# AnnSeidel/genometools

Measured on AMD Instinct MI355X. Metric: Gbp/s ESA build (suf+lcp+bwt), 3 Gbp DNA, 1/2/4/8 MI355X; bit-exact vs CPU, higher is better.
Workload: dtype u64; 1 GPU; human-like DNA (2% N, 24 seqs, repeats) n=3000000000 seed=43 -suf -lcp -bwt (BASELINE.json configs[2]); parallelism=1 device, pair_suffixes=341032298, tied_suffixes=390540711, refine_rounds=9, maxbranchdepth=8256

## Files before the change

genometools_amd/csrc/esa_engine.hip:

```cpp
#include <stdarg.h>
#include <stdlib.h>
#include <chrono>
#include <functional>
#include <type_traits>
#include <vector>
#include "../../include/gtamd_esa.h"
#include "esa_prims.h"
#include "esa_devutil.h"

static thread_local char g_err[1024] = "";
void gtamd_set_error(const char *fmt, ...) {
  va_list ap;
  va_start(ap, fmt);
  vsnprintf(g_err, sizeof g_err, fmt, ap);
  va_end(ap);
}
extern "C" const char *gtamd_esa_last_error(void) { return g_err; }

extern "C" int gtamd_device_count(void) {
  GTAMD_ABI_BEGIN
  int n = 0;
  if (hipGetDeviceCount(&n) != hipSuccess) return 0;
  return n;
  GTAMD_ABI_END(0)
// ... 570 lines not shown
                              u32 numparts, u64 nblocks, u32 *__restrict__ counts) {
  const u32 r = threadIdx.x;
  if (r >= numparts) return;
  const u64 first = (u64) r * nblocks, last = first + nblocks - 1;
  counts[r] = boff[last] + bcount[last] - boff[first];
}

struct Tiles {
  u64 T;
  u32 self;
  __device__ __forceinline__ u32 owner(u64 q, u64 *off) const {
    const u64 d = q / T;
    *off = q - d * T;
    return (u32) d;
  }
};

struct OwnerOfKey {
  const u64 *keys;
  const u32 *vals;
  const u8 *owner;
  u64 *keys_out;
  u32 *vals_out;
  __device__ __forceinline__ u32 dest(u64 j) const {
    return owner[keys[j] >> (64 - PART_BITS)];
  }
  __device__ __forceinline__ void local(u64) const {}
  __device__ __forceinline__ void emit(u64 j, u32 at) const {
    keys_out[at] = keys[j];
    vals_out[at] = vals[j];
  }
};

template <typename P> struct InitialRanks {
  const P *sa;
  const u64 *tiebits;
  const u32 *carry;
  u64 c0, index_offset;
  Tiles tl;
  P *isa;
  u32 *srec;
  const u32 *sel;
  int wb;
  __device__ __forceinline__ u32 dest(u64 j) const {
    u64 off;
    const u64 p = (u64) sa[c0 + j];
    if (sel != nullptr) {
      const u64 w = p >> wb;
      if (!((sel[w >> 5] >> (w & 31)) & 1u)) return DEST_NONE;
    }
    const u32 d = tl.owner(p, &off);
    return d == tl.self ? DEST_LOCAL : d;
  }
  __device__ __forceinline__ P rank_of(u64 i) const {
    const u64 w = i >> 6;
    const int b = (int) (i & 63);
    const u64 below = b == 63 ? ~0ull : ((2ull << b) - 1ull);
    const u64 z = ~tiebits[w] & below;
    const u64 head = z ? w * 64 + (u64) (63 - __clzll((long long) z)) : (u64) carry[w];
    return (P) (index_offset + head);
  }
  __device__ __forceinline__ void local(u64 j) const {
    u64 off;
    (void) tl.owner((u64) sa[c0 + j], &off);
    isa[off] = rank_of(c0 + j);
  }
  __device__ __forceinline__ void emit(u64 j, u32 at) const {
    u64 off;
    (void) tl.owner((u64) sa[c0 + j], &off);
    const u64 r = (u64) rank_of(c0 + j);
    u32 *rec = srec + (u64) at * (1 + sizeof(P) / 4);
    rec[0] = (u32) off;
    rec[1] = (u32) r;
    if (sizeof(P) == 8) rec[2] = (u32) (r >> 32);
  }
};

template <typename P> struct FilteredRanks {
  const P *fpos;
  const u32 *fhead;
  u64 index_offset;
  Tiles tl;
  P *isa;
  u32 *srec;
  static constexpr int RANKREC = 1 + (int) (sizeof(P) / 4);
  __device__ __forceinline__ u32 dest(u64 j) const {
    u64 off;
    const u32 d = tl.owner((u64) fpos[j], &off);
    return d == tl.self ? DEST_LOCAL : d;
  }
  __device__ __forceinline__ void local(u64 j) const {
    u64 off;
    (void) tl.owner((u64) fpos[j], &off);
// ... 427 lines not shown
__global__ __launch_bounds__(256) void k_unres_emit(
    const u64 *__restrict__ tiebits, u64 nwords, const u32 *__restrict__ blkoff,
    const u32 *__restrict__ carry, const P *__restrict__ sa,
    u32 *__restrict__ uidx0, u32 *__restrict__ uidx, P *__restrict__ upos,
    u32 *__restrict__ ugrp) {
  __shared__ u32 s_scan[4];
  const u64 w = (u64) blockIdx.x * 256 + threadIdx.x;
  u64 t = 0, u = 0;
  if (w < nwords) {
    t = tiebits[w];
    const u64 nx = w + 1 < nwords ? tiebits[w + 1] : 0ull;
    u = t | (t >> 1) | (nx << 63);
  }
  u32 tot;
  u32 j = blkoff[blockIdx.x] + block_scan_excl_sum((u32) __popcll(u), &tot, s_scan);
  if (u == 0) return;
  const u32 carryw = carry[w];
  while (u) {
    const int b = __ffsll((unsigned long long) u) - 1;
    u &= u - 1;
    const u64 i = w * 64 + b;
    const u64 below = b == 63 ? ~0ull : ((2ull << b) - 1ull);
    const u64 z = ~t & below;
    uidx0[j] = (u32) i;
    uidx[j] = (u32) i;
    upos[j] = sa[i];
    ugrp[j] = z ? (u32) (w * 64 + (63 - __clzll((long long) z))) : carryw;
    j++;
  }
}

__global__ __launch_bounds__(256) void k_heads(
    const u64 *__restrict__ tiebits, const u32 *__restrict__ carry, u64 N,
    u32 rank_offset, u32 *__restrict__ heads) {
  const u64 i0 = ((u64) blockIdx.x * 256 + threadIdx.x) * 4;
  if (i0 >= N) return;
  const u64 t = tiebits[i0 >> 6];
  u32 h[4];
  h[0] = group_head(tiebits, carry, i0);
#pragma unroll
  for (int g = 1; g < 4; g++)
    h[g] = ((t >> ((i0 + g) & 63)) & 1ull) ? h[g - 1] : (u32) (i0 + g);
  if (i0 + 4 <= N) {
    *reinterpret_cast<uint4 *>(heads + i0) =
        make_uint4(rank_offset + h[0], rank_offset + h[1], rank_offset + h[2],
                   rank_offset + h[3]);
  } else {
    for (int g = 0; g < 4 && i0 + g < N; g++) heads[i0 + g] = rank_offset + h[g];
  }
}

constexpr int RW_BITS = 15;
constexpr int RW_THREADS = 1024;

__global__ __launch_bounds__(RW_THREADS) void k_rank_window(
    const u32 *__restrict__ pos, const u32 *__restrict__ heads, u64 N, int wb,
    int split, u32 nbuckets, u32 *__restrict__ rank, const u32 *__restrict__ winlist,
    int fb, u32 nfine, u64 M) {
  __shared__ u32 s_win[1 << RW_BITS];
  u32 bucket = blockIdx.x, half = 0;
  if (split == 2) {
    bucket = (blockIdx.x >> 4) * 8u + (blockIdx.x & 7u);
    half = (blockIdx.x >> 3) & 1u;
  }
  if (bucket >= nbuckets) return;
  const int sb = wb - (split == 2 ? 1 : 0);
  const u32 smask = (1u << sb) - 1u;
  const u64 first = (u64) bucket << wb;
  const u64 total = winlist != nullptr ? M : N;
  const u64 end = first + (1ull << wb) < total ? first + (1ull << wb) : total;
  const u64 cnt = end - first;
  const u32 *bp = pos + first, *bh = heads + first;
  const u64 cnt4 = (wb >= 2) ? (cnt & ~3ull) : 0;
  for (u64 i = (u64) threadIdx.x * 4; i < cnt4; i += (u64) RW_THREADS * 4) {
    const uint4 p4 = *reinterpret_cast<const uint4 *>(bp + i);
// ... 97 lines not shown
}

constexpr int WF_THREADS = 1024;
constexpr int WF_Q = 4;
constexpr u64 WF_SPAN = (u64) WF_THREADS * 4 * WF_Q;
constexpr int WF_ITER = 8;
constexpr int WF_QUEUE = 2048;
constexpr u64 WF_LDS_MAX = 60 * 1024;
template <typename P>
__device__ __forceinline__ void wf_load4(const P *__restrict__ sa, u64 i0, u64 NL, P v[4]) {
  if (i0 + 4 <= NL) {
    if (sizeof(P) == 4) {
      const uint4 x = *reinterpret_cast<const uint4 *>(sa + i0);
      v[0] = (P) x.x; v[1] = (P) x.y; v[2] = (P) x.z; v[3] = (P) x.w;
    } else {
      const ulonglong2 v0 = *reinterpret_cast<const ulonglong2 *>(sa + i0);
      const ulonglong2 v1 = *reinterpret_cast<const ulonglong2 *>(sa + i0 + 2);
      v[0] = (P) v0.x; v[1] = (P) v0.y; v[2] = (P) v1.x; v[3] = (P) v1.y;
    }
  } else {
#pragma unroll
    for (int k = 0; k < 4; k++) v[k] = i0 + k < NL ? sa[i0 + k] : (P) 0;
  }
}
template <typename P>
static size_t wf_lds_bytes(u64 nww, bool lsel) {
  const u64 nww4 = (nww + 3) & ~3ull;
  return (size_t) ((lsel ? nww4 * 4 + nww4 : 0) + 16 + WF_QUEUE * (sizeof(P) + 2));
}
template <typename P, bool LSEL>
__global__ __launch_bounds__(WF_THREADS) __attribute__((amdgpu_waves_per_eu(8, 8))) void k_win_filter(
    const P *__restrict__ sa, u64 NL, int wb, const u32 *__restrict__ sel, u32 nww,
    const u32 *__restrict__ pref, const u64 *__restrict__ tiebits, const u32 *__restrict__ carry,
    P *__restrict__ fpos, u32 *__restrict__ fhead, u64 cap, Stats *stats) {
  extern __shared__ __attribute__((aligned(16))) u32 s_dyn[];
  __shared__ u32 s_scan[WF_THREADS / 64];
  __shared__ u32 s_base;
  const u32 nww4 = (nww + 3u) & ~3u;
  u32 *s_sel = s_dyn, *s_pref4 = s_dyn + nww4;
  P *s_qpos = reinterpret_cast<P *>(s_dyn + (LSEL ? nww4 + nww4 / 4 : 0u) + ((LSEL ? nww4 / 4 : 0u) & 1u));
  unsigned short *s_qidx = reinterpret_cast<unsigned short *>(s_qpos + WF_QUEUE);
  if (LSEL) {
    for (u32 i = threadIdx.x; i < nww4; i += WF_THREADS) s_sel[i] = i < nww ? sel[i] : 0u;
    if (pref != nullptr)
      for (u32 i = threadIdx.x; i < nww4 / 4; i += WF_THREADS) s_pref4[i] = pref[4 * i];
    __syncthreads();
  }
  const u32 *selw = LSEL ? s_sel : sel;
  for (int it = 0; it < WF_ITER; it++) {
    const u64 first = ((u64) blockIdx.x * WF_ITER + it) * WF_SPAN;
    if (first >= NL) break;
    P p[WF_Q][4];
#pragma unroll
    for (int q = 0; q < WF_Q; q++)
      wf_load4(sa, first + (u64) q * (WF_THREADS * 4) + (u64) threadIdx.x * 4, NL, p[q]);
    u32 m = 0;
#pragma unroll
    for (int q = 0; q < WF_Q; q++) {
      const u64 i0 = first + (u64) q * (WF_THREADS * 4) + (u64) threadIdx.x * 4;
#pragma unroll
      for (int k = 0; k < 4; k++) {
        const u32 w = (u32) (p[q][k] >> wb);
        if (i0 + k < NL) m |= ((selw[w >> 5] >> (w & 31)) & 1u) << (4 * q + k);
      }
    }
    u32 tot;
    const u32 excl = block_scan_excl<SCAN_SUM, WF_THREADS>((u32) __popc(m), &tot, s_scan);
// ... 8 lines not shown
      for (int q = 0; q < WF_Q; q++) {
#pragma unroll
        for (int k = 0; k < 4; k++)
          if ((m >> (4 * q + k)) & 1u) {
            if (o < (u32) WF_QUEUE) {
              s_qpos[o] = p[q][k];
              s_qidx[o] = (unsigned short) (q * (WF_THREADS * 4) + threadIdx.x * 4 + k);
            }
            o++;
          }
      }
      __syncthreads();
      if (s_base == ~0u) return;
      const u32 nq = tot - r0 < (u32) WF_QUEUE ? tot - r0 : (u32) WF_QUEUE;
      const u64 base = (u64) s_base + r0;
      for (u32 j = threadIdx.x; j < nq; j += WF_THREADS) {
        P v = s_qpos[j];
        if (pref != nullptr) {
          const u32 w = (u32) (v >> wb), x = w >> 5;
          u32 d;
          if (LSEL) {
            const uint4 g = *reinterpret_cast<const uint4 *>(s_sel + (x & ~3u));
            const u32 low = (1u << (w & 31)) - 1u, jj = x & 3u;
            d = s_pref4[x >> 2] + (u32) __popc(g.x & (jj == 0 ? low : ~0u)) +
                (u32) __popc(g.y & (jj == 1 ? low : (jj > 1 ? ~0u : 0u))) +
                (u32) __popc(g.z & (jj == 2 ? low : (jj > 2 ? ~0u : 0u))) +
                (u32) __popc(g.w & (jj == 3 ? low : 0u));
          } else {
            d = pref[x] + (u32) __popc(sel[x] & ((1u << (w & 31)) - 1u));
          }
          v = (P) (((u64) d << wb) | ((u64) v & ((1ull << wb) - 1ull)));
        }
        fpos[base + j] = v;
        fhead[base + j] = group_head(tiebits, carry, first + s_qidx[j]);
      }
      __syncthreads();
    }
  }
}

constexpr int LCP_CHUNK = 32;
constexpr u32 PAIR_SWAP = 1u << 31;

__device__ __forceinline__ u64 pair_heads(u64 t, u64 nx) {
  return ~t & ((t >> 1) | (nx << 63)) & ~((t >> 2) | (nx << 62));
}

__device__ __forceinline__ u64 small_heads(u64 t, u64 nx, int g) {
  u64 m = ~t & ~((t >> g) | (nx << (64 - g)));
  for (int k = 1; k < g; k++) m &= (t >> k) | (nx << (64 - k));
  return m;
}

__global__ __launch_bounds__(256) void k_pair_words(
    const u64 *__restrict__ tiebits, u64 nwords, u32 *__restrict__ cnt,
    u32 *__restrict__ scnt, u32 *__restrict__ rcnt, u64 *__restrict__ tiebits2) {
  __shared__ u32 s4[4];
  const u64 w = (u64) blockIdx.x * 256 + threadIdx.x;
  u32 np = 0, n3 = 0, n4 = 0;
  if (w < nwords) {
    const u64 t = tiebits[w];
    const u64 nx = w + 1 < nwords ? tiebits[w + 1] : 0ull;
    const u64 ph = pair_heads(t, nx);
    u64 prevhead = 0;
    if (w > 0) prevhead = pair_heads(tiebits[w - 1], t) >> 63;
    np = (u32) __popcll(ph);
    n3 = (u32) __popcll(small_heads(t, nx, 3));
// ... 172 lines not shown
  if (w < nwords) {
    const u64 t = tiebits[w];
    const u64 nx = w + 1 < nwords ? tiebits[w + 1] : 0ull;
    ph = pair_heads(t, nx);
  }
  u32 tot;
  u32 local = block_scan_excl_sum((u32) __popcll(ph), &tot, s_scan);
  const u32 base = off[blockIdx.x];
  const bool staged = tot <= (u32) PE_STAGE;
  while (ph) {
    const int b = __ffsll((unsigned long long) ph) - 1;
    ph &= ph - 1;
    const u64 i = w * 64 + b;
    const u64 j = (u64) base + local;
    const P a = sa[i];
    const u64 v = (sizeof(P) == 4 ? (u64) sa[i + 1] : i) | (j << 32);
    if (staged) { s_pk[local] = a; s_pv[local] = v; s_pi[local] = (u32) i; }
    else { pkey[j] = a; pval[j] = v; pidx[j] = (u32) i; }
    local++;
  }
  if (!staged) return;
  __syncthreads();
  for (u32 k = threadIdx.x; k < tot; k += 256) {
    pkey[base + k] = s_pk[k];
    pval[base + k] = s_pv[k];
    pidx[base + k] = s_pi[k];
  }
}

constexpr int PR_LINE = 16;
template <int BITS, typename P>
__global__ __launch_bounds__(256) void k_pair_resolve(
    Text t, const P *__restrict__ pkey, const u64 *__restrict__ pval, u64 nrec, u64 np,
    const u32 *__restrict__ pidx, P *__restrict__ sa, u32 *__restrict__ res, Stats *stats,
    int chunk) {
  __shared__ unsigned long long s_sum[4], s_large[4];
  __shared__ u32 s_max[4];
  const int lane = threadIdx.x & 63, w = threadIdx.x >> 6;
  unsigned long long sum = 0, nlarge = 0;
  u32 mx = 0;
  const u64 nchunks = (nrec + chunk - 1) / chunk;
  for (u64 c = (u64) blockIdx.x * 256 + threadIdx.x; c < nchunks;
       c += (u64) gridDim.x * 256) {
    constexpr int RING = 4;
    u64 ra[RING] = {0, 0, 0, 0}, rb[RING] = {0, 0, 0, 0}, rl[RING] = {0, 0, 0, 0};
    bool rf[RING] = {true, true, true, true};
    int filled = 0;
    for (int e0 = 0; e0 < chunk; e0 += PR_LINE) {
      const u64 s0 = c * chunk + e0;
      if (s0 >= nrec) break;
      P ak[PR_LINE];
      u64 ivk[PR_LINE];
      if (s0 + PR_LINE <= nrec) {
        if (sizeof(P) == 4) {
#pragma unroll
          for (int q = 0; q < PR_LINE / 4; q++) {
            const uint4 v = *reinterpret_cast<const uint4 *>(pkey + s0 + 4 * q);
            ak[4 * q] = (P) v.x; ak[4 * q + 1] = (P) v.y; ak[4 * q + 2] = (P) v.z; ak[4 * q + 3] = (P) v.w;
          }
        } else {
#pragma unroll
          for (int q = 0; q < PR_LINE / 2; q++) {
            const ulonglong2 v = *reinterpret_cast<const ulonglong2 *>(pkey + s0 + 2 * q);
            ak[2 * q] = (P) v.x; ak[2 * q + 1] = (P) v.y;
          }
        }
#pragma unroll
        for (int q = 0; q < PR_LINE / 2; q++) {
// ... 6 lines not shown
          ak[q] = s0 + q < nrec ? pkey[s0 + q] : (P) 0;
          ivk[q] = s0 + q < nrec ? pval[s0 + q] : 0ull;
        }
      }
#pragma unroll
    for (int e = 0; e < PR_LINE; e++) {
      const u64 s = s0 + e;
      if (s >= nrec || e0 + e >= chunk) continue;
      const u64 a = ak[e];
      const u64 iv = ivk[e];
      const u64 j = iv >> 32;
      const u64 b = sizeof(P) == 4 ? (iv & 0xFFFFFFFFull) : (u64) sa[(iv & 0xFFFFFFFFull) + 1];
      u64 l = 0;
      bool a_first = true, known = false;
#pragma unroll
      for (int k = 0; k < RING; k++) {
        if (k < filled && !known) {
          const u64 d = a - ra[k];
          if (b >= rb[k] && b - rb[k] == d && rl[k] >= (u64) Key<BITS>::KNOWN + d) {
            l = rl[k] - d;
            a_first = rf[k];
            known = true;
          }
        }
      }
      if (!known) l = lcp_extend_long<BITS, 4>(t, a, b, (u64) Key<BITS>::KNOWN, &a_first);
#pragma unroll
      for (int k = RING - 1; k > 0; k--) { ra[k] = ra[k - 1]; rb[k] = rb[k - 1]; rl[k] = rl[k - 1]; rf[k] = rf[k - 1]; }
      ra[0] = a; rb[0] = b; rl[0] = l; rf[0] = a_first;
      if (filled < RING) filled++;
      const u32 lv = l < 0x7FFFFFFFull ? (u32) l : 0x7FFFFFFFu;
      res[j] = lv | (a_first ? 0u : PAIR_SWAP);
      if (j < np) {
        if (!a_first) {
          const u64 i = sizeof(P) == 4 ? (u64) pidx[j] : (iv & 0xFFFFFFFFull);
          sa[i] = (P) b;
          sa[i + 1] = (P) a;
        }
        sum += lv;
        nlarge += lv >= GTAMD_LCPOVERFLOW;
        mx = lv > mx ? lv : mx;
      }
    }
    }
  }
#pragma unroll
  for (int d = 32; d >= 1; d >>= 1) {
    sum += __shfl_xor(sum, d, 64);
    nlarge += __shfl_xor(nlarge, d, 64);
    const u32 o = __shfl_xor(mx, d, 64);
    mx = o > mx ? o : mx;
  }
  if (lane == 0) { s_sum[w] = sum; s_large[w] = nlarge; s_max[w] = mx; }
  __syncthreads();
  if (threadIdx.x == 0) {
    unsigned long long S = 0, Lg = 0;
    u32 M = 0;
    for (int i = 0; i < 4; i++) {
      S += s_sum[i]; Lg += s_large[i]; M = s_max[i] > M ? s_max[i] : M;
    }
    if (S) atomicAdd(&stats->lcpsum, S);
    if (Lg) atomicAdd(&stats->numlarge, Lg);
    if (M) atomicMax(&stats->maxlcp, M);
  }
}

template <typename P>
__global__ __launch_bounds__(256) void k_pair_apply(
    const u32 *__restrict__ pidx, const u32 *__restrict__ res, u64 np,
    const P *__restrict__ sa, u64 *__restrict__ suf, u8 *__restrict__ lcp,
    u8 *__restrict__ bwt, u32 *__restrict__ lcpfull, u64 index_offset, Stats *stats) {
  for (u64 j = (u64) blockIdx.x * 256 + threadIdx.x; j < np; j += (u64) gridDim.x * 256) {
    const u64 i = pidx[j];
    const u32 r = res[j], lv = r & ~PAIR_SWAP;
    if (lcp != nullptr) {
      lcp[i + 1] = (u8) (lv < GTAMD_LCPOVERFLOW ? lv : GTAMD_LCPOVERFLOW);
      if (lv >= GTAMD_LCPOVERFLOW) lcpfull[i + 1] = lv;
    }
    if (r & PAIR_SWAP) {
      const u64 x = sa[i], y = sa[i + 1];
      if (y == 0) stats->longest = index_offset + i + 1;
      if (suf != nullptr) { suf[i] = x; suf[i + 1] = y; }
      if (bwt != nullptr) {
        const u8 b0 = bwt[i], b1 = bwt[i + 1];
        bwt[i] = b1;
        bwt[i + 1] = b0;
      }
    }
  }
}

constexpr int RT_TILE = 2048;
constexpr int RT_THREADS = 256;
constexpr int RT_PER = RT_TILE / RT_THREADS;

template <typename P> struct RoundKey {
  static constexpr int KK = sizeof(P) == 8 ? 40 : 32;
  static __device__ __forceinline__ u64 pack(u32 lg, bool open, u64 kk, u32 e) {
    return ((u64) lg << (12 + KK)) | ((u64) open << (11 + KK)) | (kk << 11) | (u64) e;
  }
  static __device__ __forceinline__ bool open(u64 key) { return (key >> (11 + KK)) & 1ull; }
};

template <typename P>
__global__ __launch_bounds__(RT_THREADS) void k_round_tile(
    const u32 *__restrict__ uidx, const P *__restrict__ upos,
    const u32 *__restrict__ ugrp, P *__restrict__ k2, u64 m,
    P *__restrict__ cv, u32 *__restrict__ hv, const u32 *__restrict__ tstart,
    u32 *__restrict__ flagbits, const P *__restrict__ rank, u64 h, u64 n) {
  using RK = RoundKey<P>;
  constexpr bool WIDE = sizeof(P) == 8;
  __shared__ u64 s_key[RT_TILE];
  __shared__ P s_pos[RT_TILE];
  __shared__ u64 s_k2w[WIDE ? RT_TILE : 1];
  __shared__ u16 s_start[RT_TILE + 2];
// ... 1812 lines not shown
    TRY(ensure_buf(c, c->tiebits2, (nwords + 2) * 8, "the tie bitmap"));
    u64 *tiebits2 = c->tiebits2.as<u64>();
    const bool no_pairs = sw.no_pairs;
    const bool no_small = no_pairs || sw.no_small_groups;
    u64 nsmall = 0, nsrec = 0;
    if (NL > 0) {
      if (no_pairs) {
        HIP_TRY(hipMemcpyAsync(tiebits2, tiebits, nwords * 8, hipMemcpyDeviceToDevice, st));
      } else {
        k_pair_words<<<(u32) nwb, 256, 0, st>>>(tiebits, nwords, pcnt, scnt, rcnt, tiebits2);
        HIP_TRY(hipGetLastError());
        TRY(scan_u32(SCAN_SUM, pcnt, poff, nwb, false, scanws, st));
        TRY(scan_u32(SCAN_SUM, scnt, soff, nwb, false, scanws, st));
        TRY(scan_u32(SCAN_SUM, rcnt, roff, nwb, false, scanws, st));
        k_total2<<<1, 1, 0, st>>>(poff, pcnt, nwb, c->d_stats);
        k_total3<<<1, 1, 0, st>>>(soff, scnt, nwb, c->d_stats);
        k_total<<<1, 1, 0, st>>>(roff, rcnt, nwb, c->d_stats);
        HIP_TRY(hipGetLastError());
        TRY(fetch_stats(c));
        npairs = c->h_stats->count2;
        nsmall = c->h_stats->count3;
        nsrec = c->h_stats->count;
      }
    }
    if (no_small || nsrec > NL / 8 || npairs + nsrec >= SINGLE_LIMIT) { nsmall = 0; nsrec = 0; }
    const u64 nrec = npairs + nsrec;
    const u64 pp = (nrec + 64 + 3) & ~3ull;
    const u64 sp = (nsmall + 64 + 3) & ~3ull;
    P *pk_a = nullptr, *pk_b = nullptr;
    u64 *pv_a = nullptr, *pv_b = nullptr;
    u32 *pidx = nullptr, *pres = nullptr, *prws = nullptr, *sidx = nullptr, *sres = nullptr,
        *slcp = nullptr, *srec = nullptr;
    u8 *ssize = nullptr;
    auto layout_p = [&](Bump &a) {
      pk_a = a.take<P>(pp); pk_b = a.take<P>(pp);
      pv_a = a.take<u64>(pp); pv_b = a.take<u64>(pp);
      pidx = a.take<u32>(pp); pres = a.take<u32>(pp);
      prws = a.take<u32>(radix_workspace_words(nrec));
      sidx = a.take<u32>(sp); sres = a.take<u32>(sp); slcp = a.take<u32>(3 * sp);
      srec = a.take<u32>(sp);
      ssize = a.take<u8>(sp);
    };
    int apply_early = sw.apply_early;
    {
      Bump sz = {nullptr, 0};
      layout_p(sz);
      fail = ensure_buf(c, c->arena_p, sz.off + 4096, "the pairs of tied suffixes") != 0;
      if (!fail && want_lcp && apply_early && nrec > 0)
        fail = ensure_buf(c, c->lcpfull_buf, (NL + 8) * 4, "the LCP values beyond the byte") != 0;
      if (R > 1) TRY(comm_allgather(c, fail, nullptr, nullptr, 0));
      else if (fail) return -1;
      Bump a = {c->arena_p.as<u8>(), 0};
      layout_p(a);
    }
    const int nb = bits_for(N - 1);
    const int nbl = bits_for(NL ? NL - 1 : 0);
    auto passes_for = [](int bits, int *ps, int *pw) -> int {
      int cnt = 0;
      for (int b = 0; b < bits; b += 8) {
        ps[cnt] = b;
        pw[cnt] = bits - b < 8 ? bits - b : 8;
        cnt++;
      }
      return cnt;
    };
    int ps[8], pw[8];
    const int pn = passes_for(nb, ps, pw);
    if (nrec > 0) {
      if (npairs > 0) {
        k_pair_emit<P><<<(u32) div_up(nwords, 256), 256, 0, st>>>(tiebits, nwords, poff, sa, pk_a,
                                                                 pv_a, pidx);
        HIP_TRY(hipGetLastError());
      }
      if (nsmall > 0) {
        k_small_emit<P><<<(u32) div_up(nwords, 256), 256, 0, st>>>(
            tiebits, nwords, soff, roff, sa, npairs, sidx, ssize, srec, pk_a, pv_a);
        HIP_TRY(hipGetLastError());
      }
      TRY(radix_sort_pairs<P, u64>(pk_a, pv_a, pk_b, pv_b, nrec, ps, pw, pn, prws, st,
                                   nullptr, nullptr));
      const P *pk_sorted = (pn & 1) ? pk_b : pk_a;
      const u64 *pv_sorted = (pn & 1) ? pv_b : pv_a;
      TRY(launch_emission());
      int pair_chunk = (int) (nrec >> 20 < 16 ? 16 : (nrec >> 20 > 128 ? 128 : nrec >> 20));
      if (sw.pair_chunk > 0) pair_chunk = sw.pair_chunk;
      pair_chunk = (pair_chunk + PR_LINE - 1) / PR_LINE * PR_LINE;
      k_pair_resolve<BITS, P><<<stride_grid(div_up(div_up(nrec, (u64) pair_chunk), 256)), 256, 0, st>>>(
          c->text, pk_sorted, pv_sorted, nrec, npairs, pidx, sa, pres, c->d_stats, pair_chunk);
      HIP_TRY(hipGetLastError());
      if (nsmall > 0) {
        k_small_combine<P><<<(u32) div_up(nsmall, 256), 256, 0, st>>>(
            sidx, ssize, srec, pres, nsmall, sa, tiebits2, sres, slcp, c->d_stats);
        HIP_TRY(hipGetLastError());
      }
    }
    u32 *lcpfull = nullptr;
    if (want_lcp && apply_early && nrec > 0) lcpfull = c->lcpfull_buf.as<u32>();
    if (nrec == 0) apply_early = 0;
    u64 apply_wgs = 256;
    {
      int cus = 0;
      if (hipDeviceGetAttribute(&cus, hipDeviceAttributeMultiprocessorCount, c->device) == hipSuccess && cus > 0)
        apply_wgs = (u64) cus;
    }
    if (sw.apply_wgs > 0) apply_wgs = sw.apply_wgs;
    const bool apply_wgs_given = sw.apply_wgs_given;
    auto launch_apply = [&](hipStream_t s) -> int {
      u64 cap = ~0ull;
      if (apply_early == 1) cap = apply_wgs;
      else if (apply_early == 2 && m0 > 0) {
        cap = apply_wgs;
        if (!apply_wgs_given) {
          const double need = 7.7e-8 * (double) npairs + 2.85e-7 * (double) nsmall;
          const double have = 1.25 * 4.0e-7 * (double) m0 + 0.5;
          if (need > have) cap = (u64) ((double) apply_wgs * (need / have));
        }
      }
      if (npairs > 0) {
        const u64 g = div_up(npairs, 256);
        k_pair_apply<P><<<(u32) (g < cap ? g : cap), 256, 0, s>>>(
            pidx, pres, npairs, sa, d_suf, d_lcp, d_bwt, lcpfull, index_offset, c->d_stats);
        HIP_TRY(hipGetLastError());
      }
      if (nsmall > 0) {
        const u64 g = div_up(nsmall, 256);
        k_small_apply<P><<<(u32) (g < cap ? g : cap), 256, 0, s>>>(
            sidx, sres, slcp, nsmall, sa, d_suf, d_lcp, d_bwt, lcpfull, index_offset, c->d_stats);
        HIP_TRY(hipGetLastError());
      }
      return 0;
    };
    auto apply_beside = [&]() -> int {
      HIP_TRY(hipEventRecord(c->ev_sorted, st));
      HIP_TRY(hipStreamWaitEvent(c->st2, c->ev_sorted, 0));
      TRY(launch_apply(c->st2));
      HIP_TRY(hipEventRecord(c->ev_applied, c->st2));
      return 0;
    };
    if (apply_early == 1) TRY(apply_beside());
    TRY(tie_words(tiebits2));
    m0 = c->h_stats->count;
    const u64 smalldone = c->h_stats->smalldone;
    u64 anyleft = m0;
    if (R > 1) {
      std::vector<u64> all(R);
      TRY(comm_allgather(c, 0, &m0, all.data(), 8));
      anyleft = 0;
      for (u32 r = 0; r < R; r++) anyleft += all[r];
    }
    if (debug)
      fprintf(stderr, "gtamd: part %u: %llu tied with a neighbour, %llu pairs, %llu small groups "
              "(%llu entries settled), %llu left\n",
              c->part, (unsigned long long) numties, (unsigned long long) npairs,
              (unsigned long long) nsmall, (unsigned long long) smalldone,
              (unsigned long long) m0);
    const u64 mp = (m0 + 64 + 3) & ~3ull;
    const u64 ISA_CHUNK = 1ull << 27;
    const u64 ichunk = NL < ISA_CHUNK ? NL : ISA_CHUNK;
    const u64 xm = dist ? (ichunk > mp ? ichunk : mp) : 0;
    u64 xrecv_n = (u64) R * ISA_CHUNK > anyleft ? (u64) R * ISA_CHUNK : anyleft;
    if (xrecv_n > Tn) xrecv_n = Tn;
    xrecv_n += 64;
    P *upos = nullptr, *upos2 = nullptr, *cvo = nullptr,
      *k2 = nullptr, *fk2 = nullptr, *fk2s_a = nullptr, *fk2s_b = nullptr, *fpos = nullptr,
// ... 97 lines not shown
      const int wmax = sw.rank_window_bits;
      const u32 *spos = reinterpret_cast<const u32 *>(sa);
      const bool heads_array = bits_for(N - 1) <= wmax;
      int pb = nb > wmax ? nb - wmax : 0;
      if (pb > 16) pb = 16;
      const int wb = nb - pb;
      if (wb > wmax + 1) {
        gtamd_set_error("rank table: %d position bits do not fit two passes and a "
                        "%d-bit window", nb, wmax);
        return -1;
      }
      const int split = wb > wmax ? 2 : 1;
      const int fb = wmax < RW_FINE ? wmax : RW_FINE;
      rk_wb = fb;
      rk_nwin = div_up(N, 1ull << fb);
      const u64 nww = rk_nwin / 32 + 2;
      const bool all_windows = sw.rank_all_windows || pb == 0;
      u32 *w_pref = nullptr;
      if (!all_windows) {
        TRY(ensure_buf(c, c->winbuf, (4 * nww + rk_nwin + 16) * 4, "the rank windows"));
        w_need = c->winbuf.as<u32>(); w_built = w_need + nww; w_sel = w_built + nww;
        w_pref = w_sel + nww;
        w_list = w_pref + nww;
        HIP_TRY(hipMemsetAsync(w_need, 0, 2 * nww * 4, st));
        rk_h0 = (u64) K::KNOWN << 9;
        if (rk_h0 > (3ull << wb)) rk_h0 = 3ull << wb;
        if (m0 > 0) {
          k_win_mark<P><<<(u32) div_up(m0, 256), 256, 0, st>>>(upos, m0, 0, rk_h0, fb, rk_nwin,
                                                              w_need);
          HIP_TRY(hipGetLastError());
        }
        rk_windows = true;
      }
      const GroupHeadValues headgen = {tiebits2, carry, nwords, 0u};
      build_rank = [=, &rk_windows, &rank_built](bool first) -> int {
        u64 nsel = 0;
        if (rk_windows) {
          k_win_select<<<1, 1024, 0, st>>>(w_need, w_built, nww, w_sel, w_list, w_pref, c->d_stats);
          HIP_TRY(hipGetLastError());
          TRY(fetch_stats(c));
          nsel = c->h_stats->count;
          if (nsel == 0) return 0;
          if (first && nsel * 2 > rk_nwin) rk_windows = false;
          if (debug)
            fprintf(stderr, "gtamd: rank table: %llu of %llu windows of 2^%d positions%s\n",
                    (unsigned long long) nsel, (unsigned long long) rk_nwin, fb,
                    rk_windows ? "" : " -> whole table");
        }
        if (!rk_windows) {
          if (heads_array) {
            k_heads<<<(u32) div_up(NL, 1024), 256, 0, st>>>(tiebits2, carry, NL, 0u, heads);
            HIP_TRY(hipGetLastError());
          }
          const u32 *wpos = spos, *whead = heads;
          if (pb > 8) {
            const int s0 = nb - pb, w0 = pb - 8, s1 = nb - 8, w1 = 8;
            if (heads_array)
              TRY(radix_partition_u32(spos, heads, ppos, phead, NL, s0, w0, pws, st));
            else
              TRY(radix_pass_group_heads(spos, headgen, ppos, phead, NL, s0, w0, pws, st));
            TRY(radix_sort_pairs<u32, u32>(ppos, phead, qpos, qhead, NL, &s1, &w1, 1, pws, st,
                                           nullptr, nullptr));
            wpos = qpos; whead = qhead;
          } else if (pb > 0) {
            const int s0 = nb - pb, w0 = pb;
            if (heads_array)
              TRY(radix_partition_u32(spos, heads, ppos, phead, NL, s0, w0, pws, st));
            else
              TRY(radix_pass_group_heads(spos, headgen, ppos, phead, NL, s0, pb, pws, st));
            wpos = ppos; whead = phead;
          }
          const u32 nbuckets = (u32) div_up(NL, 1ull << wb);
          const u32 grid = split == 2 ? ((nbuckets + 7u) / 8u) * 16u : nbuckets;
          k_rank_window<<<grid, RW_THREADS, 0, st>>>(wpos, whead, NL, wb, split, nbuckets, rank32,
                                                     nullptr, 0, 0u, 0);
          HIP_TRY(hipGetLastError());
          rank_built = NL;
          return 0;
        }
        HIP_TRY(hipMemsetAsync(&c->d_stats->count, 0, 4, st));
        if ((nww + 4) * 5 <= WF_LDS_MAX && !wf_global) {
          HIP_TRY(hipFuncSetAttribute(reinterpret_cast<const void *>(&k_win_filter<u32, true>),
                                      hipFuncAttributeMaxDynamicSharedMemorySize,
                                      (int) wf_lds_bytes<u32>(nww, true)));
          k_win_filter<u32, true><<<(u32) div_up(NL, WF_SPAN * WF_ITER), WF_THREADS, wf_lds_bytes<u32>(nww, true), st>>>(
              spos, NL, fb, w_sel, (u32) nww, w_pref, tiebits2, carry, ppos, phead, ~0ull, c->d_stats);
        } else
          k_win_filter<u32, false><<<(u32) div_up(NL, WF_SPAN * WF_ITER), WF_THREADS, wf_lds_bytes<u32>(nww, false), st>>>(
              spos, NL, fb, w_sel, (u32) nww, w_pref, tiebits2, carry, ppos, phead, ~0ull, c->d_stats);
        HIP_TRY(hipGetLastError());
        TRY(fetch_stats(c));
        const u64 M = c->h_stats->count;
        if (M == 0) return 0;
        rank_built += M;
        int mb = bits_for(((u64) nsel << fb) - 1);
        if (mb < fb) mb = fb;
        int pbm = mb > wmax ? mb - wmax : 0;
        if (pbm > 16) pbm = 16;
        const int wbm = mb - pbm;
        const int splitm = wbm > wmax ? 2 : 1;
        const u32 *wpos = ppos, *whead = phead;
        if (pbm > 8) {
          const int s0 = mb - pbm, w0 = pbm - 8, s1 = mb - 8, w1 = 8;
          TRY(radix_partition_u32(ppos, phead, qpos, qhead, M, s0, w0, pws, st));
          TRY(radix_sort_pairs<u32, u32>(qpos, qhead, ppos, phead, M, &s1, &w1, 1, pws, st,
                                         nullptr, nullptr));
        } else if (pbm > 0) {
          const int s0 = mb - pbm, w0 = pbm;
          TRY(radix_partition_u32(ppos, phead, qpos, qhead, M, s0, w0, pws, st));
          wpos = qpos; whead = qhead;
        }
        const u32 nbuckets = (u32) div_up(M, 1ull << wbm);
        const u32 grid = splitm == 2 ? ((nbuckets + 7u) / 8u) * 16u : nbuckets;
        k_rank_window<<<grid, RW_THREADS, 0, st>>>(wpos, whead, N, wbm, splitm, nbuckets, rank32,
                                                   w_list, fb, (u32) nsel, M);
        HIP_TRY(hipGetLastError());
        return 0;
      };
      TRY(build_rank(true));
    }
    std::vector<u64> qcounts(R), ucounts(R), zero(R, 0);
    const size_t GW = 2 * (size_t) R + 2;
// ... 40 lines not shown
            HIP_TRY(hipStreamSynchronize(st));
            HIP_TRY(hipMemcpy(h_need.data(), w_need, dw_nww * 4, hipMemcpyDeviceToHost));
          }
          TRY(comm_allgather(c, fail, h_need.data(), h_all.data(), (u32) (dw_nww * 4)));
          agreed = 1;
          u64 fresh = 0, all = 0;
          for (u64 w = 0; w < dw_nww; w++) {
            u32 x = 0;
            for (u32 r = 0; r < R; r++) x |= h_all[(size_t) r * dw_nww + w];
            x &= ~h_built[w];
            h_need[w] = x;
            h_built[w] |= x;
            fresh += (u64) __builtin_popcount(x);
            all += (u64) __builtin_popcount(h_built[w]);
          }
          if (debug)
            fprintf(stderr, "gtamd: part %u: ranks of %llu more windows of 2^%d positions travel "
                    "(%llu of %llu so far)\n", c->part, (unsigned long long) fresh, rk_wb,
                    (unsigned long long) all, (unsigned long long) rk_nwin);
          if (fresh == 0) return 0;
          HIP_TRY(hipMemcpyAsync(w_sel, h_need.data(), dw_nww * 4, hipMemcpyHostToDevice, st));
          HIP_TRY(hipMemcpyAsync(w_built, h_built.data(), dw_nww * 4, hipMemcpyHostToDevice, st));
          d_sel = w_sel;
        }
        bool listed = false;
        u64 M = 0;
        if (!fail && d_sel != nullptr && NL > 0 && list_cap > 0) {
          HIP_TRY(hipMemsetAsync(&c->d_stats->count, 0, 8, st));
          if ((dw_nww + 4) * 5 <= WF_LDS_MAX && !wf_global) {
            HIP_TRY(hipFuncSetAttribute(reinterpret_cast<const void *>(&k_win_filter<P, true>),
                                        hipFuncAttributeMaxDynamicSharedMemorySize,
                                        (int) wf_lds_bytes<P>(dw_nww, true)));
            k_win_filter<P, true><<<(u32) div_up(NL, WF_SPAN * WF_ITER), WF_THREADS, wf_lds_bytes<P>(dw_nww, true), st>>>(
                sa, NL, rk_wb, d_sel, (u32) dw_nww, nullptr, tiebits2, carry, fpos, fhead, list_cap, c->d_stats);
          } else
            k_win_filter<P, false><<<(u32) div_up(NL, WF_SPAN * WF_ITER), WF_THREADS, wf_lds_bytes<P>(0, false), st>>>(
                sa, NL, rk_wb, d_sel, 0u, nullptr, tiebits2, carry, fpos, fhead, list_cap, c->d_stats);
          HIP_TRY(hipGetLastError());
          TRY(fetch_stats(c));
          listed = c->h_stats->count2 == 0;
          M = c->h_stats->count;
        }
        const u64 items = listed ? M : NL, per = listed ? (xm ? xm : 1) : ISA_CHUNK;
        u64 chunks = div_up(items, per);
        if (R > 1 || !agreed) {
          std::vector<u64> all(R);
          TRY(comm_allgather(c, agreed ? 0 : fail, &chunks, all.data(), 8));
          for (u32 r = 0; r < R; r++) chunks = all[r] > chunks ? all[r] : chunks;
        }
        for (u64 ch = 0; ch < chunks; ch++) {
          const u64 c0 = ch * per < items ? ch * per : items;
          const u64 cm = items - c0 < per ? items - c0 : per;
          if (listed) {
            FilteredRanks<P> fr;
            fr.fpos = fpos + c0; fr.fhead = fhead + c0; fr.index_offset = index_offset; fr.tl = tl;
            fr.isa = isa; fr.srec = xmsg;
            TRY(dest_count(c, fr, cm, xdest_q, xbc_q, xbo_q, scanws2, 0));
            HIP_TRY(hipMemcpyAsync(c->h_counts, c->d_counts, DEST_MAXPARTS * 4,
                                   hipMemcpyDeviceToHost, st));
            TRY(dest_place(c, fr, cm, xdest_q, xbo_q));
          } else {
            InitialRanks<P> ir;
            ir.sa = sa; ir.tiebits = tiebits2; ir.carry = carry; ir.c0 = c0;
            ir.index_offset = index_offset; ir.tl = tl; ir.isa = isa; ir.srec = xmsg;
            ir.sel = d_sel; ir.wb = rk_wb;
            TRY(dest_count(c, ir, cm, xdest_q, xbc_q, xbo_q, scanws2, 0));
            HIP_TRY(hipMemcpyAsync(c->h_counts, c->d_counts, DEST_MAXPARTS * 4,
                                   hipMemcpyDeviceToHost, st));
            TRY(dest_place(c, ir, cm, xdest_q, xbo_q));
          }
          HIP_TRY(hipStreamSynchronize(st));
          std::vector<u64> sc(R), rc(R), mat((size_t) R * R);
          for (u32 r = 0; r < R; r++) sc[r] = c->h_counts[r];
          TRY(comm_allgather(c, 0, sc.data(), mat.data(), R * 8));
          u64 nrecv = 0;
          for (u32 s = 0; s < R; s++) { rc[s] = mat[(size_t) s * R + c->part]; nrecv += rc[s]; }
          int toobig = 0;
          for (u32 q = 0; q < R && !toobig; q++) {
            u64 tot = 0;
            for (u32 s = 0; s < R; s++) tot += mat[(size_t) s * R + q];
            const u64 first_q = (u64) q * tl.T < N ? (u64) q * tl.T : N;
            const u64 tile_q = first_q + tl.T < N ? tl.T : N - first_q;
            if (tot > tile_q) toobig = 1;
          }
          if (toobig || nrecv + 64 > xrecv_n) {
            gtamd_set_error("rank exchange: %llu ranks for a tile of %llu positions",
                            (unsigned long long) nrecv, (unsigned long long) Tn);
            return -1;
          }
          TRY(comm_alltoallv(c, xmsg, sc.data(), xrecv_msg, rc.data(), (u32) (4 * RANKREC), "first ranks"));
          if (nrecv > 0) {
            k_isa_store_rec<P><<<(u32) div_up(nrecv, 256), 256, 0, st>>>(xrecv_msg, nrecv, isa);
            HIP_TRY(hipGetLastError());
          }
        }
        return 0;
      };
      TRY(send_ranks());
// ... 464 lines not shown
```

genometools_amd/csrc/esa_prims.h:

```cpp
#pragma once
#include "esa_common.h"

enum { SCAN_SUM = 0, SCAN_MAX = 1 };

u64 scan_workspace_words(u64 n);
int scan_u32(int op, const u32 *in, u32 *out, u64 n, bool inclusive, u32 *ws,
             hipStream_t st);

u64 radix_workspace_words(u64 n);
template <typename K, typename V>
int radix_sort_pairs(K *keys_a, V *vals_a, K *keys_b, V *vals_b, u64 n,
                     const int *shifts, const int *widths, int npasses,
                     u32 *ws, hipStream_t st, hipEvent_t *ev_pairs,
                     int *n_ev);

int radix_scan_tile_hist(u32 *ws, u64 n, hipStream_t st);
u64 radix_rows_workspace_words(u64 nrows);
int radix_scan_tile_rows(u32 *hist, u32 nrows, u32 *scanws, hipStream_t st);

struct GroupHeadValues {
  const u64 *tiebits;
  const u32 *carry;
  u64 nwords;
  u32 offset;
};
int radix_pass_group_heads(const u32 *keys_a, GroupHeadValues gen, u32 *keys_b,
                           u32 *vals_b, u64 n, int shift, int width, u32 *ws,
                           hipStream_t st);

int radix_partition_u32(const u32 *keys_a, const u32 *vals_a, u32 *keys_b, u32 *vals_b, u64 n,
                        int shift, int width, u32 *ws, hipStream_t st);
```

genometools_amd/csrc/esa_prims.hip:

```cpp
#include "esa_prims.h"
#include "esa_devutil.h"

namespace {

constexpr int SC_ITEMS = 16;
constexpr int SC_TILE = SC_THREADS * SC_ITEMS;

template <int OP>
__global__ __launch_bounds__(SC_THREADS) void k_scan_reduce(
    const u32 *__restrict__ in, u64 n, u32 *__restrict__ blocksum) {
  __shared__ u32 lds4[4];
  const u64 base = (u64) blockIdx.x * SC_TILE + (u64) threadIdx.x * SC_ITEMS;
  u32 acc = 0;
#pragma unroll
  for (int i = 0; i < SC_ITEMS; i++) {
    u64 idx = base + i;
    if (idx < n) acc = sc_op<OP>(acc, in[idx]);
  }
  u32 tot;
  (void) block_scan_excl<OP>(acc, &tot, lds4);
  if (threadIdx.x == 0) blocksum[blockIdx.x] = tot;
}

template <int OP, bool INCLUSIVE>
// ... 192 lines not shown
    const u32 v = hist[(u64) t * RADIX + threadIdx.x];
    hist[(u64) t * RADIX + threadIdx.x] = run;
    run += v;
  }
}

__device__ __forceinline__ u32 xcd_tile(u32 b, u32 ntiles) {
  const u32 per = (ntiles + 7u) >> 3;
  return (b & 7u) * per + (b >> 3);
}

typedef __attribute__((address_space(3))) volatile u16 lds_vu16;

struct ReadValues {
  static constexpr bool active = false;
  __device__ __forceinline__ void prefetch(u64, int, u64 &, u32 &) const {}
  __device__ __forceinline__ u32 make(u64, u64, u32) const { return 0; }
};
struct MakeGroupHeads {
  static constexpr bool active = true;
  GroupHeadValues g;
  __device__ __forceinline__ void prefetch(u64 wave_first, int lane, u64 &t, u32 &c) const {
    if (lane < RS_ITEMS) {
      u64 w = (wave_first >> 6) + (u64) lane;
      if (w >= g.nwords) w = g.nwords - 1;
      t = g.tiebits[w];
      c = g.carry[w];
    }
  }
  __device__ __forceinline__ u32 make(u64 i, u64 t, u32 c) const {
    const int b = (int) (i & 63);
    const u64 below = b == 63 ? ~0ull : ((2ull << b) - 1ull);
    const u64 z = ~t & below;
    return g.offset + (z ? ((u32) i & ~63u) + (63u - (u32) __clzll((long long) z)) : c);
  }
};

template <bool FULL, typename K, typename V, typename VG = ReadValues>
__device__ __forceinline__ void rs_scatter_tile(
    const K *__restrict__ keys_in, const V *__restrict__ vals_in,
    K *__restrict__ keys_out, V *__restrict__ vals_out, const u32 valid, int shift,
    u32 mask, u32 gbase, K *s_key, V *s_val, u16 *s_cnt_generic , u32 *s_obase,
    const VG vg = VG(), u64 first = 0 ) {
  lds_vu16 *s_cnt = (lds_vu16 *) s_cnt_generic;
  const int tid = threadIdx.x, lane = tid & 63, w = tid >> 6;
  u32 *s_scan = reinterpret_cast<u32 *>(s_key);
  K key[RS_ITEMS];
  V val[RS_ITEMS];
  u32 rk[RS_ITEMS];
  u64 vg_t = 0;
  u32 vg_c = 0;
  if (VG::active) vg.prefetch(first + (u64) w * RS_WAVE_CHUNK, lane, vg_t, vg_c);
#pragma unroll
  for (int j = 0; j < RS_ITEMS; j++) {
    const u32 e = (u32) w * RS_WAVE_CHUNK + (u32) j * 64 + lane;
    const u64 gen_t = VG::active ? __shfl(vg_t, j, 64) : 0ull;
    const u32 gen_c = VG::active ? __shfl(vg_c, j, 64) : 0u;
    if (FULL || e < valid) {
      key[j] = keys_in[e];
      val[j] = VG::active ? (V) vg.make(first + e, gen_t, gen_c) : vals_in[e];
    } else {
      key[j] = (K) ~(K) 0;
      val[j] = 0;
    }
  }
  __syncthreads();
  lds_vu16 *cnt_w = s_cnt + w * RADIX;
// ... 311 lines not shown
```

Baseline: 23.51 Gbp/s.

## Encode pair swaps as bitmask and apply lazily instead of scattering into SA

Pair resolution no longer writes swapped suffixes back into the suffix array with scattered stores. A new kernel builds a per-word up/down swap bitmask, and every group-head/rank computation (k_heads, win_filter, InitialRanks, radix group-head generator) adjusts the head by ±1 using it. The final apply step swaps the outputs itself. This removes the random SA writes at the cost of an extra small kernel, a 16-byte load per head computation and an extra buffer.

```diff
diff --git a/genometools_amd/csrc/esa_engine.hip b/genometools_amd/csrc/esa_engine.hip
--- a/genometools_amd/csrc/esa_engine.hip
+++ b/genometools_amd/csrc/esa_engine.hip
@@ -626,6 +626,13 @@
   }
 };
 
+__device__ __forceinline__ u32 swap_head(const u64 *swp, u64 i, u32 head) {
+  if (swp == nullptr) return head;
+  const ulonglong2 s = *reinterpret_cast<const ulonglong2 *>(swp + 2 * (i >> 6));
+  const int b = (int) (i & 63);
+  return head + (u32) ((s.x >> b) & 1ull) - (u32) ((s.y >> b) & 1ull);
+}
+
 template <typename P> struct InitialRanks {
   const P *sa;
   const u64 *tiebits;
@@ -636,6 +643,7 @@
   u32 *srec;
   const u32 *sel;
   int wb;
+  const u64 *swp;
   __device__ __forceinline__ u32 dest(u64 j) const {
     u64 off;
     const u64 p = (u64) sa[c0 + j];
@@ -652,7 +660,7 @@
     const u64 below = b == 63 ? ~0ull : ((2ull << b) - 1ull);
     const u64 z = ~tiebits[w] & below;
     const u64 head = z ? w * 64 + (u64) (63 - __clzll((long long) z)) : (u64) carry[w];
-    return (P) (index_offset + head);
+    return (P) (index_offset + swap_head(swp, i, (u32) head));
   }
   __device__ __forceinline__ void local(u64 j) const {
     u64 off;
@@ -1146,7 +1154,7 @@
 
 __global__ __launch_bounds__(256) void k_heads(
     const u64 *__restrict__ tiebits, const u32 *__restrict__ carry, u64 N,
-    u32 rank_offset, u32 *__restrict__ heads) {
+    u32 rank_offset, const u64 *__restrict__ swp, u32 *__restrict__ heads) {
   const u64 i0 = ((u64) blockIdx.x * 256 + threadIdx.x) * 4;
   if (i0 >= N) return;
   const u64 t = tiebits[i0 >> 6];
@@ -1155,6 +1163,14 @@
 #pragma unroll
   for (int g = 1; g < 4; g++)
     h[g] = ((t >> ((i0 + g) & 63)) & 1ull) ? h[g - 1] : (u32) (i0 + g);
+  if (swp != nullptr) {
+    const ulonglong2 sw = *reinterpret_cast<const ulonglong2 *>(swp + 2 * (i0 >> 6));
+#pragma unroll
+    for (int g = 0; g < 4; g++) {
+      const int b = (int) ((i0 + g) & 63);
+      h[g] += (u32) ((sw.x >> b) & 1ull) - (u32) ((sw.y >> b) & 1ull);
+    }
+  }
   if (i0 + 4 <= N) {
     *reinterpret_cast<uint4 *>(heads + i0) =
         make_uint4(rank_offset + h[0], rank_offset + h[1], rank_offset + h[2],
@@ -1318,7 +1334,8 @@
 __global__ __launch_bounds__(WF_THREADS) __attribute__((amdgpu_waves_per_eu(8, 8))) void k_win_filter(
     const P *__restrict__ sa, u64 NL, int wb, const u32 *__restrict__ sel, u32 nww,
     const u32 *__restrict__ pref, const u64 *__restrict__ tiebits, const u32 *__restrict__ carry,
-    P *__restrict__ fpos, u32 *__restrict__ fhead, u64 cap, Stats *stats) {
+    const u64 *__restrict__ swp, P *__restrict__ fpos, u32 *__restrict__ fhead, u64 cap,
+    Stats *stats) {
   extern __shared__ __attribute__((aligned(16))) u32 s_dyn[];
   __shared__ u32 s_scan[WF_THREADS / 64];
   __shared__ u32 s_base;
@@ -1393,7 +1410,8 @@
           v = (P) (((u64) d << wb) | ((u64) v & ((1ull << wb) - 1ull)));
         }
         fpos[base + j] = v;
-        fhead[base + j] = group_head(tiebits, carry, first + s_qidx[j]);
+        const u64 i = first + s_qidx[j];
+        fhead[base + j] = swap_head(swp, i, group_head(tiebits, carry, i));
       }
       __syncthreads();
     }
@@ -1632,8 +1650,7 @@
 template <int BITS, typename P>
 __global__ __launch_bounds__(256) void k_pair_resolve(
     Text t, const P *__restrict__ pkey, const u64 *__restrict__ pval, u64 nrec, u64 np,
-    const u32 *__restrict__ pidx, P *__restrict__ sa, u32 *__restrict__ res, Stats *stats,
-    int chunk) {
+    const P *__restrict__ sa, u32 *__restrict__ res, Stats *stats, int chunk) {
   __shared__ unsigned long long s_sum[4], s_large[4];
   __shared__ u32 s_max[4];
   const int lane = threadIdx.x & 63, w = threadIdx.x >> 6;
@@ -1706,11 +1723,6 @@
       const u32 lv = l < 0x7FFFFFFFull ? (u32) l : 0x7FFFFFFFu;
       res[j] = lv | (a_first ? 0u : PAIR_SWAP);
       if (j < np) {
-        if (!a_first) {
-          const u64 i = sizeof(P) == 4 ? (u64) pidx[j] : (iv & 0xFFFFFFFFull);
-          sa[i] = (P) b;
-          sa[i + 1] = (P) a;
-        }
         sum += lv;
         nlarge += lv >= GTAMD_LCPOVERFLOW;
         mx = lv > mx ? lv : mx;
@@ -1737,6 +1749,31 @@
     if (Lg) atomicAdd(&stats->numlarge, Lg);
     if (M) atomicMax(&stats->maxlcp, M);
   }
+}
+
+__global__ __launch_bounds__(256) void k_pair_swapbits(
+    const u64 *__restrict__ tiebits, u64 nwords, const u32 *__restrict__ off,
+    const u32 *__restrict__ res, u64 *__restrict__ swp) {
+  __shared__ u32 s_scan[4];
+  const u64 w = (u64) blockIdx.x * 256 + threadIdx.x;
+  u64 t = 0, ph = 0;
+  if (w < nwords) {
+    t = tiebits[w];
+    const u64 nx = w + 1 < nwords ? tiebits[w + 1] : 0ull;
+    ph = pair_heads(t, nx);
+  }
+  u32 tot;
+  const u32 j0 = off[blockIdx.x] + block_scan_excl_sum((u32) __popcll(ph), &tot, s_scan);
+  if (w >= nwords) return;
+  u64 up = 0, down = 0;
+  if (w > 0 && (pair_heads(tiebits[w - 1], t) >> 63) && (res[j0 - 1] & PAIR_SWAP)) down = 1;
+  u32 j = j0;
+  for (u64 h = ph; h; h &= h - 1) {
+    const int b = __ffsll((unsigned long long) h) - 1;
+    if (res[j++] & PAIR_SWAP) up |= 1ull << b;
+  }
+  down |= up << 1;
+  *reinterpret_cast<ulonglong2 *>(swp + 2 * w) = make_ulonglong2(up, down);
 }
 
 template <typename P>
@@ -1753,8 +1790,8 @@
     }
     if (r & PAIR_SWAP) {
       const u64 x = sa[i], y = sa[i + 1];
-      if (y == 0) stats->longest = index_offset + i + 1;
-      if (suf != nullptr) { suf[i] = x; suf[i + 1] = y; }
+      if (x == 0) stats->longest = index_offset + i + 1;
+      if (suf != nullptr) { suf[i] = y; suf[i + 1] = x; }
       if (bwt != nullptr) {
         const u8 b0 = bwt[i], b1 = bwt[i + 1];
         bwt[i] = b1;
@@ -3633,6 +3670,7 @@
     u32 *pidx = nullptr, *pres = nullptr, *prws = nullptr, *sidx = nullptr, *sres = nullptr,
         *slcp = nullptr, *srec = nullptr;
     u8 *ssize = nullptr;
+    u64 *swp = nullptr;
     auto layout_p = [&](Bump &a) {
       pk_a = a.take<P>(pp); pk_b = a.take<P>(pp);
       pv_a = a.take<u64>(pp); pv_b = a.take<u64>(pp);
@@ -3641,6 +3679,7 @@
       sidx = a.take<u32>(sp); sres = a.take<u32>(sp); slcp = a.take<u32>(3 * sp);
       srec = a.take<u32>(sp);
       ssize = a.take<u8>(sp);
+      swp = a.take<u64>(npairs > 0 ? 2 * nwords + 8 : 0);
     };
     int apply_early = sw.apply_early;
     {
@@ -3687,8 +3726,12 @@
       if (sw.pair_chunk > 0) pair_chunk = sw.pair_chunk;
       pair_chunk = (pair_chunk + PR_LINE - 1) / PR_LINE * PR_LINE;
       k_pair_resolve<BITS, P><<<stride_grid(div_up(div_up(nrec, (u64) pair_chunk), 256)), 256, 0, st>>>(
-          c->text, pk_sorted, pv_sorted, nrec, npairs, pidx, sa, pres, c->d_stats, pair_chunk);
+          c->text, pk_sorted, pv_sorted, nrec, npairs, sa, pres, c->d_stats, pair_chunk);
       HIP_TRY(hipGetLastError());
+      if (npairs > 0) {
+        k_pair_swapbits<<<(u32) nwb, 256, 0, st>>>(tiebits, nwords, poff, pres, swp);
+        HIP_TRY(hipGetLastError());
+      }
       if (nsmall > 0) {
         k_small_combine<P><<<(u32) div_up(nsmall, 256), 256, 0, st>>>(
             sidx, ssize, srec, pres, nsmall, sa, tiebits2, sres, slcp, c->d_stats);
@@ -3731,6 +3774,7 @@
       }
       return 0;
     };
+    const u64 *pair_swp = npairs > 0 ? swp : nullptr;
     auto apply_beside = [&]() -> int {
       HIP_TRY(hipEventRecord(c->ev_sorted, st));
       HIP_TRY(hipStreamWaitEvent(c->st2, c->ev_sorted, 0));
@@ -3894,7 +3938,7 @@
         }
         rk_windows = true;
       }
-      const GroupHeadValues headgen = {tiebits2, carry, nwords, 0u};
+      const GroupHeadValues headgen = {tiebits2, carry, nwords, 0u, pair_swp};
       build_rank = [=, &rk_windows, &rank_built](bool first) -> int {
         u64 nsel = 0;
         if (rk_windows) {
@@ -3911,7 +3955,7 @@
         }
         if (!rk_windows) {
           if (heads_array) {
-            k_heads<<<(u32) div_up(NL, 1024), 256, 0, st>>>(tiebits2, carry, NL, 0u, heads);
+            k_heads<<<(u32) div_up(NL, 1024), 256, 0, st>>>(tiebits2, carry, NL, 0u, pair_swp, heads);
             HIP_TRY(hipGetLastError());
           }
           const u32 *wpos = spos, *whead = heads;
@@ -3946,10 +3990,12 @@
                                       hipFuncAttributeMaxDynamicSharedMemorySize,
                                       (int) wf_lds_bytes<u32>(nww, true)));
           k_win_filter<u32, true><<<(u32) div_up(NL, WF_SPAN * WF_ITER), WF_THREADS, wf_lds_bytes<u32>(nww, true), st>>>(
-              spos, NL, fb, w_sel, (u32) nww, w_pref, tiebits2, carry, ppos, phead, ~0ull, c->d_stats);
+              spos, NL, fb, w_sel, (u32) nww, w_pref, tiebits2, carry, pair_swp, ppos, phead, ~0ull,
+              c->d_stats);
         } else
           k_win_filter<u32, false><<<(u32) div_up(NL, WF_SPAN * WF_ITER), WF_THREADS, wf_lds_bytes<u32>(nww, false), st>>>(
-              spos, NL, fb, w_sel, (u32) nww, w_pref, tiebits2, carry, ppos, phead, ~0ull, c->d_stats);
+              spos, NL, fb, w_sel, (u32) nww, w_pref, tiebits2, carry, pair_swp, ppos, phead, ~0ull,
+              c->d_stats);
         HIP_TRY(hipGetLastError());
         TRY(fetch_stats(c));
         const u64 M = c->h_stats->count;
@@ -4056,10 +4102,12 @@
                                         hipFuncAttributeMaxDynamicSharedMemorySize,
                                         (int) wf_lds_bytes<P>(dw_nww, true)));
             k_win_filter<P, true><<<(u32) div_up(NL, WF_SPAN * WF_ITER), WF_THREADS, wf_lds_bytes<P>(dw_nww, true), st>>>(
-                sa, NL, rk_wb, d_sel, (u32) dw_nww, nullptr, tiebits2, carry, fpos, fhead, list_cap, c->d_stats);
+                sa, NL, rk_wb, d_sel, (u32) dw_nww, nullptr, tiebits2, carry, pair_swp, fpos, fhead,
+                list_cap, c->d_stats);
           } else
             k_win_filter<P, false><<<(u32) div_up(NL, WF_SPAN * WF_ITER), WF_THREADS, wf_lds_bytes<P>(0, false), st>>>(
-                sa, NL, rk_wb, d_sel, 0u, nullptr, tiebits2, carry, fpos, fhead, list_cap, c->d_stats);
+                sa, NL, rk_wb, d_sel, 0u, nullptr, tiebits2, carry, pair_swp, fpos, fhead, list_cap,
+                c->d_stats);
           HIP_TRY(hipGetLastError());
           TRY(fetch_stats(c));
           listed = c->h_stats->count2 == 0;
@@ -4087,7 +4135,7 @@
             InitialRanks<P> ir;
             ir.sa = sa; ir.tiebits = tiebits2; ir.carry = carry; ir.c0 = c0;
             ir.index_offset = index_offset; ir.tl = tl; ir.isa = isa; ir.srec = xmsg;
-            ir.sel = d_sel; ir.wb = rk_wb;
+            ir.sel = d_sel; ir.wb = rk_wb; ir.swp = pair_swp;
             TRY(dest_count(c, ir, cm, xdest_q, xbc_q, xbo_q, scanws2, 0));
             HIP_TRY(hipMemcpyAsync(c->h_counts, c->d_counts, DEST_MAXPARTS * 4,
                                    hipMemcpyDeviceToHost, st));
diff --git a/genometools_amd/csrc/esa_prims.h b/genometools_amd/csrc/esa_prims.h
--- a/genometools_amd/csrc/esa_prims.h
+++ b/genometools_amd/csrc/esa_prims.h
@@ -23,6 +23,7 @@
   const u32 *carry;
   u64 nwords;
   u32 offset;
+  const u64 *swp;
 };
 int radix_pass_group_heads(const u32 *keys_a, GroupHeadValues gen, u32 *keys_b,
                            u32 *vals_b, u64 n, int shift, int width, u32 *ws,
diff --git a/genometools_amd/csrc/esa_prims.hip b/genometools_amd/csrc/esa_prims.hip
--- a/genometools_amd/csrc/esa_prims.hip
+++ b/genometools_amd/csrc/esa_prims.hip
@@ -248,7 +248,12 @@
     const int b = (int) (i & 63);
     const u64 below = b == 63 ? ~0ull : ((2ull << b) - 1ull);
     const u64 z = ~t & below;
-    return g.offset + (z ? ((u32) i & ~63u) + (63u - (u32) __clzll((long long) z)) : c);
+    u32 h = g.offset + (z ? ((u32) i & ~63u) + (63u - (u32) __clzll((long long) z)) : c);
+    if (g.swp != nullptr) {
+      const ulonglong2 s = *reinterpret_cast<const ulonglong2 *>(g.swp + 2 * (i >> 6));
+      h += (u32) ((s.x >> b) & 1ull) - (u32) ((s.y >> b) & 1ull);
+    }
+    return h;
   }
 };
 
```

Result: faster. 24.68 Gbp/s, median of 6 (+5.0%).
